# edwardyehuang/iSeg

Measured on AMD Instinct MI355X. Metric: train_images_per_sec (ConvNeXt-T+ASPP 512x512 crop, fwd+bwd+AdamW, whole job), higher is better.
Workload: dtype bf16

## Files before the change

### iseg_amd/csrc/mlp_fused.hip

```cpp
#include "common.h"
#include "iseg_hip.h"
#include "mlp_common.h"
#include <stdlib.h>

namespace {

typedef __attribute__((ext_vector_type(16))) float f32x16;
typedef __attribute__((address_space(3))) void* lds_void_ptr;
typedef const __attribute__((address_space(1))) void* glb_void_ptr;

constexpr int OUT_SLAB = 32 * 36 * 4;

template <int C, int SUB, int WAVES, int NIMG, int NSTAGES> struct MlpGeom {
    static constexpr int NS = NSTAGES;
    static constexpr int HID = 4 * C, KK = C / 16, CB = C / 32;
    static constexpr int IMG = C * 64;
    static constexpr int SLAB = NIMG * IMG;
    static constexpr int STAGE = SUB * SLAB;
    static constexpr int PIECES = STAGE / 1024;
    static constexpr int PLO = PIECES / WAVES, NHI = PIECES % WAVES, PHI = PLO + (NHI ? 1 : 0);
    static constexpr int NST = HID / (32 * SUB);
    static constexpr int RING = NS * STAGE > WAVES * OUT_SLAB ? NS * STAGE : WAVES * OUT_SLAB;
    static constexpr int LDS = RING + HID * 4;
    static_assert(C % 32 == 0 && STAGE % 1024 == 0 && HID % (32 * SUB) == 0 && PLO >= 1 && NST >= NS - 1 && NS >= 2 && LDS <= 160 * 1024, "geometry");
};

__device__ __forceinline__ bf16x8 lds_frag(const char* p) { return *reinterpret_cast<const bf16x8*>(p); }

template <class G, int WAVES> struct RingFeeder {
    const char* src;
    int wid;
    __device__ __forceinline__ RingFeeder(const void* tiled, int wid_, int lane) : src((const char*)tiled + wid_ * 1024 + lane * 16), wid(wid_) {}
    __device__ __forceinline__ void issue(char* smem, int stage) {
        char* dst = smem + stage * G::STAGE + wid * 1024;
#pragma unroll
        for (int i = 0; i < G::PLO; ++i)
            __builtin_amdgcn_global_load_lds((glb_void_ptr)(src + i * WAVES * 1024), (lds_void_ptr)(dst + i * WAVES * 1024), 16, 0, 0);
        if (G::NHI && wid < G::NHI)
            __builtin_amdgcn_global_load_lds((glb_void_ptr)(src + G::PLO * WAVES * 1024), (lds_void_ptr)(dst + G::PLO * WAVES * 1024), 16, 0, 0);
        src += G::STAGE;
    }
};


#define MLP_WAIT(N) asm volatile("s_waitcnt vmcnt(%0)" ::"n"(N) : "memory")

template <int C, int SUB, int WAVES, int NSTAGES>
__global__ __launch_bounds__(64 * WAVES) __attribute__((amdgpu_waves_per_eu(C == 96 ? 4 : (C == 192 ? 2 : 1)))) void convnext_mlp_fwd_kernel(const bf16_t* __restrict__ Y, const void* __restrict__ FW,
                                                               const float* __restrict__ b1, const float* __restrict__ b2,
                                                               const float* __restrict__ gamma, const float* __restrict__ rowscale,
                                                               int64_t rows_per_group, const bf16_t* __restrict__ R, bf16_t* __restrict__ O,
                                                               int64_t M, MlpLayerNorm ln) {
    using G = MlpGeom<C, SUB, WAVES, 2, NSTAGES>;
    constexpr int HID = G::HID, KK = G::KK, CB = G::CB, IMG = G::IMG, SLAB = G::SLAB, STAGE = G::STAGE, NST = G::NST, NS = G::NS;
    extern __shared__ __attribute__((aligned(1024))) char smem[];
    float* const b1s = reinterpret_cast<float*>(smem + G::RING);

    const int tid = threadIdx.x, lane = tid & 63, wid = tid >> 6;
    const int r = lane & 31, h = lane >> 5;
    const int64_t m0 = (int64_t)blockIdx.x * (32 * WAVES) + wid * 32;

    bf16x8 yf[KK];
    {
        int64_t row = m0 + r;
        row = row < M ? row : M - 1;
        const bf16_t* yp = Y + row * C + 8 * h;
#ifdef ISEG_ABL_MLP_NOIO
#pragma unroll
        for (int kk = 0; kk < KK; ++kk)
#pragma unroll
            for (int u = 0; u < 8; ++u) yf[kk][u] = (bf16_t)(0.01f * (float)((lane + kk + u) & 15));
        (void)yp;
#else
#pragma unroll
        for (int kk = 0; kk < KK; ++kk) yf[kk] = *reinterpret_cast<const bf16x8*>(yp + 16 * kk);
#endif
        if (ln.gamma) mlp_layernorm_rows<KK>(yf, ln, m0 + r < M ? m0 + r : -1, h, C);
    }
    for (int i = tid; i < HID; i += 64 * WAVES) b1s[i] = b1[i];
#pragma unroll
    for (int kk = 0; kk < KK; ++kk) asm volatile("" ::"v"(yf[kk]));

    RingFeeder<G, WAVES> feed(FW, wid, lane);

    f32x16 acc[CB];
#pragma unroll
    for (int cb = 0; cb < CB; ++cb)
// ... 17 lines not shown
        for (int sub = 0; sub < SUB; ++sub) {
            const int f0 = sub * (KK + 2 * CB);
            f32x16 hacc;
            {
                const float* bb = b1s + 32 * (kt * SUB + sub) + 4 * h;
#pragma unroll
                for (int i = 0; i < 4; ++i) {
                    const float4 v = __builtin_bit_cast(float4, lds_frag(reinterpret_cast<const char*>(bb + 8 * i)));
                    hacc[4 * i] = v.x;
                    hacc[4 * i + 1] = v.y;
                    hacc[4 * i + 2] = v.z;
                    hacc[4 * i + 3] = v.w;
                }
            }
#pragma unroll
            for (int kk = 0; kk < KK; ++kk) {
                hacc = __builtin_amdgcn_mfma_f32_32x32x16_bf16(take(f0 + kk), yf[kk], hacc, 0, 0, 0);
                __builtin_amdgcn_sched_barrier(0);
            }
            bf16x8 gf[2];
#pragma unroll
            for (int j = 0; j < 16; ++j) gf[j >> 3][j & 7] = (bf16_t)gelu_poly(hacc[j]);
            __builtin_amdgcn_sched_barrier(0);
#pragma unroll
            for (int cb = 0; cb < CB; ++cb)
#pragma unroll
                for (int s = 0; s < 2; ++s) {
                    acc[cb] = __builtin_amdgcn_mfma_f32_32x32x16_bf16(take(f0 + KK + 2 * cb + s), gf[s], acc[cb], 0, 0, 0);
                    __builtin_amdgcn_sched_barrier(0);
                }
        }
    };

#pragma unroll
    for (int p = 0; p < NS - 1; ++p) feed.issue(smem, p);
    int stage = 0, fill = NS - 1;
    for (int kt = 0; kt < NST; ++kt) {
        if (NST - 1 - kt >= NS - 2) {
            if (G::NHI && wid < G::NHI) MLP_WAIT((NS - 2) * G::PHI);
            else MLP_WAIT((NS - 2) * G::PLO);
        } else {
            MLP_WAIT(0);
        }
        asm volatile("s_waitcnt lgkmcnt(0)" ::: "memory");
        __builtin_amdgcn_s_barrier();
        asm volatile("" ::: "memory");
        if (kt + NS - 1 < NST) feed.issue(smem, fill);
        compute(stage, kt);
        stage = stage + 1 == NS ? 0 : stage + 1;
        fill = fill + 1 == NS ? 0 : fill + 1;
    }
    asm volatile("s_waitcnt lgkmcnt(0)" ::: "memory");
    __builtin_amdgcn_s_barrier();
    asm volatile("" ::: "memory");

    float* const slab = reinterpret_cast<float*>(smem + wid * OUT_SLAB);
    const int er = lane >> 1, eh = lane & 1;
    const int64_t m = m0 + er;
    float rs = 1.f;
    if (rowscale && m < M) rs = rowscale[m / rows_per_group];
#pragma unroll
    for (int cb = 0; cb < CB; ++cb) {
#pragma unroll
        for (int i = 0; i < 4; ++i)
            *reinterpret_cast<float4*>(slab + r * 36 + 8 * i + 4 * h) = make_float4(acc[cb][4 * i], acc[cb][4 * i + 1], acc[cb][4 * i + 2], acc[cb][4 * i + 3]);
        float v[16];
#pragma unroll
        for (int i = 0; i < 4; ++i) {
            const float4 t = *reinterpret_cast<const float4*>(slab + er * 36 + 16 * eh + 4 * i);
            v[4 * i] = t.x;
            v[4 * i + 1] = t.y;
            v[4 * i + 2] = t.z;
            v[4 * i + 3] = t.w;
        }
        if (m < M) {
            const int c0 = 32 * cb + 16 * eh;
            float res[16], bb[16], gg[16];
#ifdef ISEG_ABL_MLP_NOIO
#pragma unroll
            for (int u = 0; u < 16; ++u) res[u] = 0.f;
#else
            load8<bf16_t>(R + m * C + c0, res);
            load8<bf16_t>(R + m * C + c0 + 8, res + 8);
// ... 15 lines not shown
#endif
            {
                store8<bf16_t>(O + m * C + c0, v);
                store8<bf16_t>(O + m * C + c0 + 8, v + 8);
            }
        }
    }
}

__device__ __forceinline__ uint32_t pack_bf16x2(float lo, float hi) {
    typedef __attribute__((ext_vector_type(2))) __bf16 bf16x2;
    bf16x2 v;
    v[0] = (bf16_t)lo;
    v[1] = (bf16_t)hi;
    return __builtin_bit_cast(uint32_t, v);
}

__device__ __forceinline__ void acc_to_row_pieces(const float* v, uint4& p0, uint4& p1) {
    uint32_t d[8];
#pragma unroll
    for (int i = 0; i < 8; ++i) d[i] = pack_bf16x2(v[2 * i], v[2 * i + 1]);
#pragma unroll
    for (int pr = 0; pr < 2; ++pr)
#pragma unroll
        for (int w = 0; w < 2; ++w) {
            auto sw = __builtin_amdgcn_permlane32_swap(d[4 * pr + w], d[4 * pr + 2 + w], false, false);
            d[4 * pr + w] = sw[0];
            d[4 * pr + 2 + w] = sw[1];
        }
    p0 = make_uint4(d[0], d[1], d[2], d[3]);
    p1 = make_uint4(d[4], d[5], d[6], d[7]);
}

template <int C, int SUB, int WAVES, int NSTAGES, bool STORE, bool LNB = false>
__global__ __launch_bounds__(64 * WAVES) void convnext_mlp_bwd_kernel(const bf16_t* __restrict__ Y, const bf16_t* __restrict__ D,
                                                                      const float* __restrict__ rowscale, int64_t rows_per_group,
                                                                      const void* __restrict__ BW, const float* __restrict__ b1,
                                                                      bf16_t* __restrict__ Gout, bf16_t* __restrict__ DHout,
                                                                      bf16_t* __restrict__ DY, int64_t M, MlpLayerNorm ln,
                                                                      float* __restrict__ ln_partials) {
    using G = MlpGeom<C, SUB, WAVES, 3, NSTAGES>;
    constexpr int HID = G::HID, KK = G::KK, CB = G::CB, IMG = G::IMG, SLAB = G::SLAB, STAGE = G::STAGE, NST = G::NST, NS = G::NS;
    constexpr int STORES = STORE ? 4 * SUB : 0;
    extern __shared__ __attribute__((aligned(1024))) char smem[];
    float* const b1s = reinterpret_cast<float*>(smem + G::RING);

    const int tid = threadIdx.x, lane = tid & 63, wid = tid >> 6;
    const int r = lane & 31, h = lane >> 5;
    const int64_t m0 = (int64_t)blockIdx.x * (32 * WAVES) + wid * 32;
    const bool active = m0 < M;

    bf16x8 yf[KK], df[KK];
    {
        int64_t row = m0 + r;
        row = row < M ? row : M - 1;
        const bf16_t* yp = Y + row * C + 8 * h;
        const bf16_t* dp = D + row * C + 8 * h;
#pragma unroll
        for (int kk = 0; kk < KK; ++kk) {
            yf[kk] = *reinterpret_cast<const bf16x8*>(yp + 16 * kk);
            df[kk] = *reinterpret_cast<const bf16x8*>(dp + 16 * kk);
        }
        if (ln.gamma) mlp_layernorm_apply_rows<KK>(yf, ln, row, h);
        if (rowscale) {
            const float rs = rowscale[row / rows_per_group];
#pragma unroll
            for (int kk = 0; kk < KK; ++kk)
#pragma unroll
                for (int u = 0; u < 8; ++u) df[kk][u] = (bf16_t)((float)df[kk][u] * rs);
        }
    }
    for (int i = tid; i < HID; i += 64 * WAVES) b1s[i] = b1[i];
#pragma unroll
    for (int kk = 0; kk < KK; ++kk) asm volatile("" ::"v"(yf[kk]), "v"(df[kk]));

    RingFeeder<G, WAVES> feed(BW, wid, lane);
// ... 50 lines not shown
#pragma unroll
            for (int j = 0; j < 16; ++j) {
                float gd;
                if constexpr (STORE) gelu_sig_both(hacc[j], gv[j], gd);
                else gd = gelu_poly_grad(hacc[j]);
                dv[j] = dacc[j] * gd;
            }
            bf16x8 hf[2];
#pragma unroll
            for (int j = 0; j < 16; ++j) hf[j >> 3][j & 7] = (bf16_t)dv[j];
            __builtin_amdgcn_sched_barrier(0);
#pragma unroll
            for (int cb = 0; cb < CB; ++cb)
#pragma unroll
                for (int s = 0; s < 2; ++s) {
                    acc[cb] = __builtin_amdgcn_mfma_f32_32x32x16_bf16(take(f0 + 2 * KK + 2 * cb + s), hf[s], acc[cb], 0, 0, 0);
                    __builtin_amdgcn_sched_barrier(0);
                }
            if (STORE) {
                uint4 g0, g1, d0, d1;
                acc_to_row_pieces(gv, g0, g1);
                acc_to_row_pieces(dv, d0, d1);
                if (row_ok) {
                    const int64_t o = row_o + 32 * (kt * SUB + sub);
                    *reinterpret_cast<uint4*>(Gout + o) = g0;
                    *reinterpret_cast<uint4*>(Gout + o + 16) = g1;
                    *reinterpret_cast<uint4*>(DHout + o) = d0;
                    *reinterpret_cast<uint4*>(DHout + o + 16) = d1;
                }
            }
        }
    };

#pragma unroll
    for (int p = 0; p < NS - 1; ++p) feed.issue(smem, p);
    int stage = 0, fill = NS - 1;
    for (int kt = 0; kt < NST; ++kt) {
        {
            const bool more = NST - 1 - kt >= NS - 2;
            const bool hi = G::NHI && wid < G::NHI;
#define MLP_WAIT_BWD(S_)                                                     \
    do {                                                                     \
        if (more) {                                                          \
            if (hi) MLP_WAIT((NS - 2) * G::PHI + (S_));                      \
            else MLP_WAIT((NS - 2) * G::PLO + (S_));                         \
        } else {                                                             \
            MLP_WAIT(S_);                                                    \
        }                                                                    \
    } while (0)
            if (!active || kt == 0) MLP_WAIT_BWD(0);
            else if (kt == 1) MLP_WAIT_BWD(STORES);
            else MLP_WAIT_BWD(2 * STORES);
#undef MLP_WAIT_BWD
        }
        asm volatile("s_waitcnt lgkmcnt(0)" ::: "memory");
        __builtin_amdgcn_s_barrier();
        asm volatile("" ::: "memory");
        if (kt + NS - 1 < NST) feed.issue(smem, fill);
        if (active) compute(stage, kt);
        stage = stage + 1 == NS ? 0 : stage + 1;
        fill = fill + 1 == NS ? 0 : fill + 1;
    }
    asm volatile("s_waitcnt lgkmcnt(0)" ::: "memory");
    __builtin_amdgcn_s_barrier();
    asm volatile("" ::: "memory");

    float* const slab = reinterpret_cast<float*>(smem + wid * OUT_SLAB);
    const int er = lane >> 1, eh = lane & 1;
    const int64_t m = m0 + er;
    auto exchange = [&](int cb, float* v) {
#pragma unroll
        for (int i = 0; i < 4; ++i)
            *reinterpret_cast<float4*>(slab + r * 36 + 8 * i + 4 * h) = make_float4(acc[cb][4 * i], acc[cb][4 * i + 1], acc[cb][4 * i + 2], acc[cb][4 * i + 3]);
#pragma unroll
        for (int i = 0; i < 4; ++i) {
            const float4 t = *reinterpret_cast<const float4*>(slab + er * 36 + 16 * eh + 4 * i);
            v[4 * i] = t.x;
            v[4 * i + 1] = t.y;
            v[4 * i + 2] = t.z;
            v[4 * i + 3] = t.w;
        }
    };
    if constexpr (!LNB) {
#pragma unroll
        for (int cb = 0; cb < CB; ++cb) {
            float v[16];
            exchange(cb, v);
            if (m < M) {
                const int c0 = 32 * cb + 16 * eh;
                store8<bf16_t>(DY + m * C + c0, v);
                store8<bf16_t>(DY + m * C + c0 + 8, v + 8);
            }
        }
    } else {
// ... 122 lines not shown
__global__ void convnext_weight_prep_batched_kernel(const int64_t* __restrict__ table) {
    const int64_t* e = table + 8 * blockIdx.y;
    const int first = blockIdx.x * blockDim.x + threadIdx.x, stride = gridDim.x * blockDim.x;
    if (e[0] == 1) {
        mlp_prep_elements(reinterpret_cast<const float*>(e[1]), reinterpret_cast<const float*>(e[2]), reinterpret_cast<const float*>(e[3]),
                          reinterpret_cast<bf16_t*>(e[4]), reinterpret_cast<bf16_t*>(e[5]), (int)e[6], first, stride);
    } else if (e[0] == 2) {
        const float* wa = reinterpret_cast<const float*>(e[1]);
        const float* wb = reinterpret_cast<const float*>(e[2]);
        const float* ba = reinterpret_cast<const float*>(e[3]);
        const float* bb = reinterpret_cast<const float*>(e[5]);
        const int Cc = (int)e[6], na = (int)(e[7] & 0xFFFFF), nb = (int)((e[7] >> 20) & 0xFFFFF), ld = (int)(e[7] >> 40);
        bf16_t* rowcat = reinterpret_cast<bf16_t*>(e[4]);
        bf16_t* tr = rowcat + (int64_t)Cc * ld;
        float* bias = reinterpret_cast<float*>(tr + (int64_t)Cc * ld);
        const int64_t total = (int64_t)Cc * ld;
        for (int64_t i = first; i < total; i += stride) {
            const int c = (int)(i / ld), j = (int)(i % ld);
            const float v = j < na ? wa[(int64_t)c * na + j] : (j < na + nb ? wb[(int64_t)c * nb + (j - na)] : 0.f);
            rowcat[i] = (bf16_t)v;
            tr[(int64_t)j * Cc + c] = (bf16_t)v;
        }
        for (int j = first; j < ld; j += stride) bias[j] = j < na ? (ba ? ba[j] : 0.f) : (j < na + nb ? (bb ? bb[j - na] : 0.f) : 0.f);
    } else {
        const float* src = reinterpret_cast<const float*>(e[1]);
        const float* g = reinterpret_cast<const float*>(e[3]);
        bf16_t* dst = reinterpret_cast<bf16_t*>(e[4]);
        const int cols = (int)e[6];
        const int64_t total = e[7] * cols;
        for (int64_t i = first; i < total; i += stride) dst[i] = (bf16_t)(src[i] * g[i % cols]);
    }
}

template <int C, int SUB, int WAVES, int NSTAGES>
int launch_mlp_fwd(const void* y2, const void* FW, const float* b1, const float* b2, const float* gamma, const float* rowscale,
                   int64_t rows_per_group, const void* residual, void* out, int64_t M, const MlpLayerNorm& ln, hipStream_t s) {
    using G = MlpGeom<C, SUB, WAVES, 2, NSTAGES>;
    static const bool raised = [] {
        return hipFuncSetAttribute(reinterpret_cast<const void*>(&convnext_mlp_fwd_kernel<C, SUB, WAVES, NSTAGES>),
                                   hipFuncAttributeMaxDynamicSharedMemorySize, G::LDS) == hipSuccess;
    }();
    (void)raised;
    const int grid = (int)ceil_div64(M, 32 * WAVES);
    hipLaunchKernelGGL((convnext_mlp_fwd_kernel<C, SUB, WAVES, NSTAGES>), dim3(grid), dim3(64 * WAVES), G::LDS, s, (const bf16_t*)y2, FW, b1, b2, gamma, rowscale,
                       rows_per_group, (const bf16_t*)residual, (bf16_t*)out, M, ln);
    return iseg_check_launch("iseg_convnext_mlp_fwd");
}

template <int C, int SUB, int WAVES, int NSTAGES, bool STORE, bool LNB = false>
int launch_mlp_bwd(const void* y2, const void* dbr, const float* rowscale, int64_t rows_per_group, const void* BW, const float* b1, void* g,
                   void* dh, void* dy2, int64_t M, const MlpLayerNorm& ln, hipStream_t s, float* ln_partials = nullptr) {
    using G = MlpGeom<C, SUB, WAVES, 3, NSTAGES>;
    static_assert(!LNB || G::RING >= WAVES * OUT_SLAB + (WAVES * 2 + 1) * C * 4, "the column sums and gamma sit behind the epilogue slabs inside the ring");
    static const bool raised = [] {
        return hipFuncSetAttribute(reinterpret_cast<const void*>(&convnext_mlp_bwd_kernel<C, SUB, WAVES, NSTAGES, STORE, LNB>),
                                   hipFuncAttributeMaxDynamicSharedMemorySize, G::LDS) == hipSuccess;
    }();
    (void)raised;
    const int grid = (int)ceil_div64(M, 32 * WAVES);
    hipLaunchKernelGGL((convnext_mlp_bwd_kernel<C, SUB, WAVES, NSTAGES, STORE, LNB>), dim3(grid), dim3(64 * WAVES), G::LDS, s, (const bf16_t*)y2,
                       (const bf16_t*)dbr, rowscale, rows_per_group, BW, b1, (bf16_t*)g, (bf16_t*)dh, (bf16_t*)dy2, M, ln, ln_partials);
    return iseg_check_launch("iseg_convnext_mlp_bwd");
}

}

extern "C" int iseg_convnext_mlp_supported(int C, int dtype) {
    static const bool wide = [] { const char* e = getenv("ISEG_MLP_FUSED_384"); return e && atoi(e) != 0; }();
    return dtype == ISEG_BF16 && (C == 96 || C == 192 || (C == 384 && wide)) ? 1 : 0;
}

extern "C" size_t iseg_convnext_mlp_tiled_bytes(int C, int backward) { return (size_t)(backward ? 3 : 2) * 4 * C * C * 2; }

extern "C" int iseg_convnext_mlp_prep(const float* W1, const float* W2, const float* gamma, void* fw_tiled, void* bw_tiled, int C,
                                      hipStream_t stream) {
    ISEG_REQUIRE(W1 && W2 && fw_tiled && C > 0 && C % 32 == 0, "iseg_convnext_mlp_prep: bad arguments");
    const int total = (bw_tiled ? 5 : 2) * 4 * C * C;
    hipLaunchKernelGGL(convnext_mlp_prep_kernel, dim3((total + 255) / 256), dim3(256), 0, stream, W1, W2, gamma, (bf16_t*)fw_tiled,
                       (bf16_t*)bw_tiled, C);
    return iseg_check_launch("iseg_convnext_mlp_prep");
}

extern "C" int iseg_convnext_weight_prep_batched(const int64_t* table, int entries, int64_t max_elements, hipStream_t stream) {
    ISEG_REQUIRE(table && entries > 0 && max_elements > 0, "iseg_convnext_weight_prep_batched: bad arguments");
    int64_t bx = (max_elements + 255) / 256;
    if (bx > 256) bx = 256;
    hipLaunchKernelGGL(convnext_weight_prep_batched_kernel, dim3((unsigned)bx, (unsigned)entries), dim3(256), 0, stream, table);
    return iseg_check_launch("iseg_convnext_weight_prep_batched");
}

extern "C" int iseg_convnext_mlp_fwd(const void* y2, const void* fw_tiled, const float* b1, const float* b2, const float* gamma,
                                     const float* rowscale, int64_t rows_per_group, const void* residual, void* out, int64_t M, int C, int dtype,
                                     hipStream_t stream) {
    ISEG_REQUIRE(iseg_convnext_mlp_supported(C, dtype), "iseg_convnext_mlp_fwd: bf16 storage with C = 96, 192 or 384 only (C = %d, dtype = %d)", C, dtype);
    ISEG_REQUIRE(y2 && fw_tiled && b1 && b2 && residual && out && M > 0, "iseg_convnext_mlp_fwd: null operand or empty problem");
    ISEG_REQUIRE(!rowscale || rows_per_group > 0, "iseg_convnext_mlp_fwd: rowscale needs rows_per_group > 0");
    ISEG_REQUIRE((((uintptr_t)y2 | (uintptr_t)fw_tiled | (uintptr_t)residual | (uintptr_t)out | (uintptr_t)b1 | (uintptr_t)b2 | (uintptr_t)gamma) & 15) == 0,
                 "iseg_convnext_mlp_fwd: operands must be 16-byte aligned");
    const MlpLayerNorm none{};
    if (C == 96) return launch_mlp_fwd<96, 2, 8, 3>(y2, fw_tiled, b1, b2, gamma, rowscale, rows_per_group, residual, out, M, none, stream);
    if (C == 192) return launch_mlp_fwd<192, 1, 8, 3>(y2, fw_tiled, b1, b2, gamma, rowscale, rows_per_group, residual, out, M, none, stream);
    return launch_mlp_fwd<384, 1, 4, 3>(y2, fw_tiled, b1, b2, gamma, rowscale, rows_per_group, residual, out, M, none, stream);
}

extern "C" int iseg_convnext_mlp_fwd_ln(const void* y1, const float* ln_gamma, const float* ln_beta, float eps, float* mean, float* rstd,
                                        const void* fw_tiled, const float* b1, const float* b2, const float* gamma, const float* rowscale,
                                        int64_t rows_per_group, const void* residual, void* out, int64_t M, int C, int dtype, hipStream_t stream) {
    ISEG_REQUIRE(dtype == ISEG_BF16 && (C == 96 || C == 192), "iseg_convnext_mlp_fwd_ln: bf16 storage with C = 96 or 192 only (C = %d, dtype = %d)", C, dtype);
    ISEG_REQUIRE(y1 && ln_gamma && ln_beta && mean && rstd && fw_tiled && b1 && b2 && residual && out && M > 0,
                 "iseg_convnext_mlp_fwd_ln: null operand or empty problem");
    ISEG_REQUIRE(!rowscale || rows_per_group > 0, "iseg_convnext_mlp_fwd_ln: rowscale needs rows_per_group > 0");
    ISEG_REQUIRE((((uintptr_t)y1 | (uintptr_t)fw_tiled | (uintptr_t)residual | (uintptr_t)out | (uintptr_t)b1 | (uintptr_t)b2 | (uintptr_t)gamma |
                   (uintptr_t)ln_gamma | (uintptr_t)ln_beta) & 15) == 0, "iseg_convnext_mlp_fwd_ln: operands must be 16-byte aligned");
    const MlpLayerNorm ln{ln_gamma, ln_beta, mean, rstd, eps};
    if (C == 96) return launch_mlp_fwd<96, 2, 8, 3>(y1, fw_tiled, b1, b2, gamma, rowscale, rows_per_group, residual, out, M, ln, stream);
    return launch_mlp_fwd<192, 1, 8, 3>(y1, fw_tiled, b1, b2, gamma, rowscale, rows_per_group, residual, out, M, ln, stream);
}

extern "C" int iseg_convnext_mlp_bwd(const void* y2, const void* dbr, const void* bw_tiled, const float* b1, void* g, void* dh, void* dy2,
                                     int64_t M, int C, int dtype, hipStream_t stream) {
    ISEG_REQUIRE(iseg_convnext_mlp_supported(C, dtype), "iseg_convnext_mlp_bwd: bf16 storage with C = 96, 192 or 384 only (C = %d, dtype = %d)", C, dtype);
    ISEG_REQUIRE(y2 && dbr && bw_tiled && b1 && g && dh && dy2 && M > 0, "iseg_convnext_mlp_bwd: null operand or empty problem");
    ISEG_REQUIRE((((uintptr_t)y2 | (uintptr_t)dbr | (uintptr_t)bw_tiled | (uintptr_t)b1 | (uintptr_t)g | (uintptr_t)dh | (uintptr_t)dy2) & 15) == 0,
                 "iseg_convnext_mlp_bwd: operands must be 16-byte aligned");
    const MlpLayerNorm none{};
    if (C == 96) return launch_mlp_bwd<96, 2, 8, 3, true>(y2, dbr, nullptr, 0, bw_tiled, b1, g, dh, dy2, M, none, stream);
    if (C == 192) return launch_mlp_bwd<192, 1, 4, 3, true>(y2, dbr, nullptr, 0, bw_tiled, b1, g, dh, dy2, M, none, stream);
    return launch_mlp_bwd<384, 1, 4, 2, true>(y2, dbr, nullptr, 0, bw_tiled, b1, g, dh, dy2, M, none, stream);
}

extern "C" int iseg_convnext_mlp_bwd_data(const void* y2, const float* mean, const float* rstd, const float* ln_gamma, const float* ln_beta,
                                          const void* dout, const float* rowscale, int64_t rows_per_group, const void* bw_tiled,
                                          const float* b1, void* dy2, int64_t M, int C, int dtype, hipStream_t stream) {
    ISEG_REQUIRE(dtype == ISEG_BF16 && (C == 96 || C == 192), "iseg_convnext_mlp_bwd_data: bf16 storage with C = 96 or 192 only (C = %d, dtype = %d)", C, dtype);
    ISEG_REQUIRE(y2 && dout && bw_tiled && b1 && dy2 && M > 0, "iseg_convnext_mlp_bwd_data: null operand or empty problem");
    ISEG_REQUIRE(!rowscale || rows_per_group > 0, "iseg_convnext_mlp_bwd_data: rowscale needs rows_per_group > 0");
    ISEG_REQUIRE((((uintptr_t)y2 | (uintptr_t)dout | (uintptr_t)bw_tiled | (uintptr_t)b1 | (uintptr_t)dy2) & 15) == 0,
                 "iseg_convnext_mlp_bwd_data: operands must be 16-byte aligned");
    ISEG_REQUIRE(!mean || (rstd && ln_gamma && ln_beta && (((uintptr_t)ln_gamma | (uintptr_t)ln_beta) & 15) == 0),
                 "iseg_convnext_mlp_bwd_data: mean needs rstd and 16-byte aligned ln_gamma / ln_beta");
    const MlpLayerNorm ln{mean ? ln_gamma : nullptr, ln_beta, const_cast<float*>(mean), const_cast<float*>(rstd), 0.f};
    if (C == 96) return launch_mlp_bwd<96, 2, 8, 3, false>(y2, dout, rowscale, rows_per_group, bw_tiled, b1, nullptr, nullptr, dy2, M, ln, stream);
    return launch_mlp_bwd<192, 1, 4, 3, false>(y2, dout, rowscale, rows_per_group, bw_tiled, b1, nullptr, nullptr, dy2, M, ln, stream);
}

static int64_t mlp_bwd_blocks(int64_t M, int C) { return ceil_div64(M, 32 * (C == 96 ? 8 : 4)); }

extern "C" size_t iseg_convnext_mlp_bwd_data_ln_workspace_bytes(int64_t M, int C) {
    return (C == 96 || C == 192) && M > 0 ? (size_t)mlp_bwd_blocks(M, C) * 2 * C * sizeof(float) : 0;
}

extern "C" int iseg_convnext_mlp_bwd_data_ln(const void* y1, const float* mean, const float* rstd, const float* ln_gamma, const float* ln_beta,
                                             const void* dout, const float* rowscale, int64_t rows_per_group, const void* bw_tiled,
                                             const float* b1, void* dy1, float* dln_gamma, float* dln_beta, int64_t M, int C, int dtype,
                                             void* ws, size_t ws_bytes, hipStream_t stream) {
    ISEG_REQUIRE(dtype == ISEG_BF16 && (C == 96 || C == 192), "iseg_convnext_mlp_bwd_data_ln: bf16 storage with C = 96 or 192 only (C = %d, dtype = %d)", C, dtype);
    ISEG_REQUIRE(y1 && mean && rstd && ln_gamma && ln_beta && dout && bw_tiled && b1 && dy1 && dln_gamma && dln_beta && M > 0,
                 "iseg_convnext_mlp_bwd_data_ln: null operand or empty problem");
    ISEG_REQUIRE(!rowscale || rows_per_group > 0, "iseg_convnext_mlp_bwd_data_ln: rowscale needs rows_per_group > 0");
    ISEG_REQUIRE((((uintptr_t)y1 | (uintptr_t)dout | (uintptr_t)bw_tiled | (uintptr_t)b1 | (uintptr_t)dy1 | (uintptr_t)ln_gamma | (uintptr_t)ln_beta) & 15) == 0,
                 "iseg_convnext_mlp_bwd_data_ln: operands must be 16-byte aligned");
    const size_t need = iseg_convnext_mlp_bwd_data_ln_workspace_bytes(M, C);
    if (!ws || ws_bytes < need) {
        iseg_set_error("iseg_convnext_mlp_bwd_data_ln: needs %zu workspace bytes, got %zu", need, ws_bytes);
        return ISEG_ERR_WORKSPACE;
    }
    const MlpLayerNorm ln{ln_gamma, ln_beta, const_cast<float*>(mean), const_cast<float*>(rstd), 0.f};
    float* partials = (float*)ws;
    float* const arena = iseg_deferred_partials(need, dln_gamma, dln_beta, 1, stream);
    if (arena) partials = arena;
    const int rc = C == 96 ? launch_mlp_bwd<96, 2, 8, 3, false, true>(y1, dout, rowscale, rows_per_group, bw_tiled, b1, nullptr, nullptr, dy1, M, ln,
                                                                       stream, partials)
                           : launch_mlp_bwd<192, 1, 4, 3, false, true>(y1, dout, rowscale, rows_per_group, bw_tiled, b1, nullptr, nullptr, dy1, M, ln,
                                                                        stream, partials);
    if (rc != ISEG_OK) return rc;
    const int blocks = (int)mlp_bwd_blocks(M, C);
    if (arena) iseg_deferred_push(partials, blocks, 2 * C, 2 * C, dln_gamma, dln_beta, C, 1.f, stream);
    else launch_reduce_rows(partials, blocks, 2 * C, 0, 1, 2 * C, dln_gamma, dln_beta, C, 0, 1.f, 1, stream);
    return iseg_check_launch("iseg_convnext_mlp_bwd_data_ln");
}
```

Measured before the change: 1938.

## Skew fused ConvNeXt MLP pipeline to overlap GELU with next slab's MFMAs

Adds a software-pipelined (skewed) schedule to the fused ConvNeXt MLP forward and backward-data kernels. The first-layer product for the next hidden slab is issued while the GELU (or GELU-gradient) of the current slab runs, interleaved with sched_group_barrier hints, so VALU work hides behind MFMA latency. The ring-wait logic is generalized into a helper to cover reading two ring stages per iteration. The new path is on by default for C=192 forward and for backward-data, and is gated by an environment variable. The forward C=96 variant needs level 2 and also lowers the waves-per-EU hint when enabled. The cost is extra registers for the second accumulator, which may lower occupancy.

```diff
diff --git a/iseg_amd/csrc/mlp_fused.hip b/iseg_amd/csrc/mlp_fused.hip
--- a/iseg_amd/csrc/mlp_fused.hip
+++ b/iseg_amd/csrc/mlp_fused.hip
@@ -45,14 +45,65 @@
 
 #define MLP_WAIT(N) asm volatile("s_waitcnt vmcnt(%0)" ::"n"(N) : "memory")
 
-template <int C, int SUB, int WAVES, int NSTAGES>
-__global__ __launch_bounds__(64 * WAVES) __attribute__((amdgpu_waves_per_eu(C == 96 ? 4 : (C == 192 ? 2 : 1)))) void convnext_mlp_fwd_kernel(const bf16_t* __restrict__ Y, const void* __restrict__ FW,
+template <class G, int STORES, int MAXP> __device__ __forceinline__ void mlp_ring_wait(int stages, int store_iters, bool hi) {
+#define MLP_WAIT_PK(P_, K_)                                                          \
+    do {                                                                             \
+        if (hi) MLP_WAIT((P_ * G::PHI + K_ * STORES) < 63 ? P_ * G::PHI + K_ * STORES : 63); \
+        else MLP_WAIT((P_ * G::PLO + K_ * STORES) < 63 ? P_ * G::PLO + K_ * STORES : 63);    \
+    } while (0)
+#define MLP_WAIT_P(P_)                                  \
+    do {                                                \
+        if (STORES == 0 || store_iters == 0) MLP_WAIT_PK(P_, 0); \
+        else if (store_iters == 1) MLP_WAIT_PK(P_, 1);  \
+        else MLP_WAIT_PK(P_, 2);                        \
+    } while (0)
+    if (MAXP == 0 || stages == 0) MLP_WAIT_P(0);
+    else if (MAXP == 1 || stages == 1) MLP_WAIT_P(1);
+    else MLP_WAIT_P(2);
+#undef MLP_WAIT_P
+#undef MLP_WAIT_PK
+}
+
+template <class G, int STORES, bool SKEW> __device__ __forceinline__ void mlp_ring_sync(int kt, bool stores_issued) {
+    constexpr int NS = G::NS, NST = G::NST;
+    const int need = SKEW && kt + 1 < NST ? kt + 1 : kt;
+    const int issued = kt + NS - 2 < NST - 1 ? kt + NS - 2 : NST - 1;
+    const int first_store = need - (NS - 1) > 0 ? need - (NS - 1) : 0;
+    int k = stores_issued && STORES ? kt - first_store : 0;
+    k = k < 2 ? k : 2;
+    constexpr int MAXP = (SKEW ? NS - 3 : NS - 2) < 2 ? (SKEW ? NS - 3 : NS - 2) : 2;
+    static_assert(NS <= 4 || !SKEW, "mlp_ring_wait counts at most two pending stages");
+    mlp_ring_wait<G, STORES, MAXP>(issued - need, k, G::NHI && threadIdx.x / 64 < G::NHI);
+    asm volatile("s_waitcnt lgkmcnt(0)" ::: "memory");
+    __builtin_amdgcn_s_barrier();
+    asm volatile("" ::: "memory");
+}
+
+template <bool B> struct MlpFlag { static constexpr bool value = B; };
+
+#ifndef ISEG_MLP_SKEW_NS
+#define ISEG_MLP_SKEW_NS 3
+#endif
+#ifndef ISEG_MLP_SKEW_ALT
+#define ISEG_MLP_SKEW_ALT 0
+#endif
+
+constexpr int SG_VALU = 0x2, SG_MFMA = 0x8, SG_DS_READ = 0x100;
+#ifdef ISEG_MLP_NOSGB
+#define MLP_SGB(M_, N_) ((void)0)
+#else
+#define MLP_SGB(M_, N_) __builtin_amdgcn_sched_group_barrier(M_, N_, 0)
+#endif
+
+template <int C, int SUB, int WAVES, int NSTAGES, bool SKEW>
+__global__ __launch_bounds__(64 * WAVES) __attribute__((amdgpu_waves_per_eu(C == 96 ? (SKEW ? 2 : 4) : (C == 192 ? 2 : 1)))) void convnext_mlp_fwd_kernel(const bf16_t* __restrict__ Y, const void* __restrict__ FW,
                                                                const float* __restrict__ b1, const float* __restrict__ b2,
                                                                const float* __restrict__ gamma, const float* __restrict__ rowscale,
                                                                int64_t rows_per_group, const bf16_t* __restrict__ R, bf16_t* __restrict__ O,
                                                                int64_t M, MlpLayerNorm ln) {
     using G = MlpGeom<C, SUB, WAVES, 2, NSTAGES>;
     constexpr int HID = G::HID, KK = G::KK, CB = G::CB, IMG = G::IMG, SLAB = G::SLAB, STAGE = G::STAGE, NST = G::NST, NS = G::NS;
+    static_assert(!SKEW || (NS >= 3 && NST >= 2), "the skewed schedule reads two ring stages per iteration and refills a third");
     extern __shared__ __attribute__((aligned(1024))) char smem[];
     float* const b1s = reinterpret_cast<float*>(smem + G::RING);
 
@@ -136,23 +187,123 @@
         }
     };
 
+    constexpr int PER = KK + 2 * CB;
+#ifndef ISEG_MLP_SKEW_FD
+#define ISEG_MLP_SKEW_FD FD
+#endif
+    constexpr int FDS = ISEG_MLP_SKEW_FD;
+    constexpr int VALU_A = 16 * 11 + 8;
+    constexpr int VPER = (VALU_A + KK) / (KK + 1) + 11;
+    f32x16 hc;
+    auto bias = [&](int slab) {
+        f32x16 a;
+        const float* bb = b1s + 32 * slab + 4 * h;
+#pragma unroll
+        for (int i = 0; i < 4; ++i) {
+            const float4 v = __builtin_bit_cast(float4, lds_frag(reinterpret_cast<const char*>(bb + 8 * i)));
+            a[4 * i] = v.x;
+            a[4 * i + 1] = v.y;
+            a[4 * i + 2] = v.z;
+            a[4 * i + 3] = v.w;
+        }
+        return a;
+    };
+    auto first_product = [&](int stage) {
+        const char* fb = smem + stage * STAGE + fo;
+        bf16x8 win[FDS];
+#pragma unroll
+        for (int d = 0; d < FDS; ++d) win[d] = lds_frag(fb + d * 1024);
+        hc = bias(0);
+#pragma unroll
+        for (int kk = 0; kk < KK; ++kk) {
+            const bf16x8 a = win[kk % FDS];
+            if (kk + FDS < KK) win[kk % FDS] = lds_frag(fb + (kk + FDS) * 1024);
+            hc = __builtin_amdgcn_mfma_f32_32x32x16_bf16(a, yf[kk], hc, 0, 0, 0);
+            __builtin_amdgcn_sched_barrier(0);
+        }
+    };
+    auto compute_skew = [&](int stage, int kt, auto last_c) {
+        constexpr bool LAST = decltype(last_c)::value;
+        constexpr int NFS = SUB * PER - (LAST ? KK : 0);
+        const char* cur = smem + stage * STAGE + fo;
+        const char* nxt = smem + (stage + 1 == NS ? 0 : stage + 1) * STAGE + fo;
+        auto frag_at = [&](int f) {
+            const int sub = f / PER, q = f % PER;
+            const bool succ = !(LAST && sub == SUB - 1);
+            if (succ && q < KK) return lds_frag((sub + 1 < SUB ? cur + (sub + 1) * SLAB : nxt) + q * 1024);
+            return lds_frag(cur + sub * SLAB + (succ ? q : KK + q) * 1024);
+        };
+        bf16x8 win[FDS];
+#pragma unroll
+        for (int d = 0; d < FDS; ++d) win[d] = frag_at(d);
+        auto take = [&](int f) {
+            const bf16x8 a = win[f % FDS];
+            if (f + FDS < NFS) win[f % FDS] = frag_at(f + FDS);
+            return a;
+        };
+#pragma unroll
+        for (int sub = 0; sub < SUB; ++sub) {
+            const int f0 = sub * PER;
+            const bool succ = !(LAST && sub == SUB - 1);
+            bf16x8 gf[2];
+            if (succ) {
+                f32x16 hn = bias(kt * SUB + sub + 1);
+                __builtin_amdgcn_sched_barrier(0);
+#pragma unroll
+                for (int c = 0; c <= KK; ++c) {
+                    if (c > 0) hn = __builtin_amdgcn_mfma_f32_32x32x16_bf16(take(f0 + c - 1), yf[c - 1], hn, 0, 0, 0);
+#pragma unroll
+                    for (int j = 16 * c / (KK + 1); j < 16 * (c + 1) / (KK + 1); ++j) gf[j >> 3][j & 7] = (bf16_t)gelu_poly(hc[j]);
+                    if (c > 0) {
+                        MLP_SGB(SG_MFMA, 1);
+                        MLP_SGB(SG_DS_READ, 1);
+                        MLP_SGB(SG_VALU, VPER);
+                    }
+                    __builtin_amdgcn_sched_barrier(0);
+                }
+                hc = hn;
+            } else {
+#pragma unroll
+                for (int j = 0; j < 16; ++j) gf[j >> 3][j & 7] = (bf16_t)gelu_poly(hc[j]);
+                __builtin_amdgcn_sched_barrier(0);
+            }
+            const int f2 = f0 + (succ ? KK : 0);
+#pragma unroll
+            for (int cb = 0; cb < CB; ++cb)
+#pragma unroll
+                for (int s = 0; s < 2; ++s) {
+                    acc[cb] = __builtin_amdgcn_mfma_f32_32x32x16_bf16(take(f2 + 2 * cb + s), gf[s], acc[cb], 0, 0, 0);
+                    __builtin_amdgcn_sched_barrier(0);
+                }
+        }
+    };
+
 #pragma unroll
     for (int p = 0; p < NS - 1; ++p) feed.issue(smem, p);
     int stage = 0, fill = NS - 1;
-    for (int kt = 0; kt < NST; ++kt) {
-        if (NST - 1 - kt >= NS - 2) {
-            if (G::NHI && wid < G::NHI) MLP_WAIT((NS - 2) * G::PHI);
-            else MLP_WAIT((NS - 2) * G::PLO);
-        } else {
-            MLP_WAIT(0);
-        }
-        asm volatile("s_waitcnt lgkmcnt(0)" ::: "memory");
-        __builtin_amdgcn_s_barrier();
-        asm volatile("" ::: "memory");
-        if (kt + NS - 1 < NST) feed.issue(smem, fill);
-        compute(stage, kt);
-        stage = stage + 1 == NS ? 0 : stage + 1;
-        fill = fill + 1 == NS ? 0 : fill + 1;
+    if constexpr (SKEW) {
+        mlp_ring_sync<G, 0, true>(0, false);
+        if (NS - 1 < NST) feed.issue(smem, fill);
+        first_product(stage);
+        compute_skew(stage, 0, MlpFlag<false>{});
+        stage = 1, fill = 0;
+        for (int kt = 1; kt < NST - 1; ++kt) {
+            mlp_ring_sync<G, 0, true>(kt, false);
+            if (kt + NS - 1 < NST) feed.issue(smem, fill);
+            compute_skew(stage, kt, MlpFlag<false>{});
+            stage = stage + 1 == NS ? 0 : stage + 1;
+            fill = fill + 1 == NS ? 0 : fill + 1;
+        }
+        mlp_ring_sync<G, 0, true>(NST - 1, false);
+        compute_skew(stage, NST - 1, MlpFlag<true>{});
+    } else {
+        for (int kt = 0; kt < NST; ++kt) {
+            mlp_ring_sync<G, 0, false>(kt, false);
+            if (kt + NS - 1 < NST) feed.issue(smem, fill);
+            compute(stage, kt);
+            stage = stage + 1 == NS ? 0 : stage + 1;
+            fill = fill + 1 == NS ? 0 : fill + 1;
+        }
     }
     asm volatile("s_waitcnt lgkmcnt(0)" ::: "memory");
     __builtin_amdgcn_s_barrier();
@@ -234,7 +385,7 @@
     p1 = make_uint4(d[4], d[5], d[6], d[7]);
 }
 
-template <int C, int SUB, int WAVES, int NSTAGES, bool STORE, bool LNB = false>
+template <int C, int SUB, int WAVES, int NSTAGES, bool STORE, bool LNB, bool SKEW>
 __global__ __launch_bounds__(64 * WAVES) void convnext_mlp_bwd_kernel(const bf16_t* __restrict__ Y, const bf16_t* __restrict__ D,
                                                                       const float* __restrict__ rowscale, int64_t rows_per_group,
                                                                       const void* __restrict__ BW, const float* __restrict__ b1,
@@ -244,6 +395,7 @@
     using G = MlpGeom<C, SUB, WAVES, 3, NSTAGES>;
     constexpr int HID = G::HID, KK = G::KK, CB = G::CB, IMG = G::IMG, SLAB = G::SLAB, STAGE = G::STAGE, NST = G::NST, NS = G::NS;
     constexpr int STORES = STORE ? 4 * SUB : 0;
+    static_assert(!SKEW || (NS >= 3 && NST >= 2), "the skewed schedule reads two ring stages per iteration and refills a third");
     extern __shared__ __attribute__((aligned(1024))) char smem[];
     float* const b1s = reinterpret_cast<float*>(smem + G::RING);
 
@@ -360,34 +512,148 @@
         }
     };
 
+    constexpr int NP1 = 2 * KK, PER = NP1 + 2 * CB;
+    constexpr bool ALT = ISEG_MLP_SKEW_ALT;
+    constexpr int VALU_A = STORE ? 16 * 24 + 8 : 16 * 13 + 8;
+    constexpr int VPER = (VALU_A + NP1) / (NP1 + 1) + 24;
+    f32x16 hc, dc;
+    auto bias = [&](int slab) {
+        f32x16 a;
+        const float* bb = b1s + 32 * slab + 4 * h;
+#pragma unroll
+        for (int i = 0; i < 4; ++i) {
+            const float4 v = __builtin_bit_cast(float4, lds_frag(reinterpret_cast<const char*>(bb + 8 * i)));
+            a[4 * i] = v.x;
+            a[4 * i + 1] = v.y;
+            a[4 * i + 2] = v.z;
+            a[4 * i + 3] = v.w;
+        }
+        return a;
+    };
+    auto first_product = [&](int stage) {
+        const char* fb = smem + stage * STAGE + fo;
+        bf16x8 win[FD];
+#pragma unroll
+        for (int d = 0; d < FD; ++d) win[d] = lds_frag(fb + d * 1024);
+        hc = bias(0);
+#pragma unroll
+        for (int j = 0; j < 16; ++j) dc[j] = 0.f;
+#pragma unroll
+        for (int f = 0; f < NP1; ++f) {
+            const bf16x8 a = win[f % FD];
+            if (f + FD < NP1) win[f % FD] = lds_frag(fb + (f + FD) * 1024);
+            if (f < KK) hc = __builtin_amdgcn_mfma_f32_32x32x16_bf16(a, yf[f], hc, 0, 0, 0);
+            else dc = __builtin_amdgcn_mfma_f32_32x32x16_bf16(a, df[f - KK], dc, 0, 0, 0);
+            __builtin_amdgcn_sched_barrier(0);
+        }
+    };
+    auto compute_skew = [&](int stage, int kt, auto last_c) {
+        constexpr bool LAST = decltype(last_c)::value;
+        constexpr int NFS = SUB * PER - (LAST ? NP1 : 0);
+        const char* cur = smem + stage * STAGE + fo;
+        const char* nxt = smem + (stage + 1 == NS ? 0 : stage + 1) * STAGE + fo;
+        auto frag_at = [&](int f) {
+            const int sub = f / PER, q = f % PER;
+            const bool succ = !(LAST && sub == SUB - 1);
+            if (succ && q < NP1) return lds_frag((sub + 1 < SUB ? cur + (sub + 1) * SLAB : nxt) + (ALT ? (q & 1 ? KK : 0) + q / 2 : q) * 1024);
+            return lds_frag(cur + sub * SLAB + (succ ? q : NP1 + q) * 1024);
+        };
+        bf16x8 win[FD];
+#pragma unroll
+        for (int d = 0; d < FD; ++d) win[d] = frag_at(d);
+        auto take = [&](int f) {
+            const bf16x8 a = win[f % FD];
+            if (f + FD < NFS) win[f % FD] = frag_at(f + FD);
+            return a;
+        };
+#pragma unroll
+        for (int sub = 0; sub < SUB; ++sub) {
+            const int f0 = sub * PER;
+            const bool succ = !(LAST && sub == SUB - 1);
+            float gv[16], dv[16];
+            bf16x8 hf[2];
+            auto chain = [&](int j0, int j1) {
+#pragma unroll
+                for (int j = j0; j < j1; ++j) {
+                    float gd;
+                    if constexpr (STORE) gelu_sig_both(hc[j], gv[j], gd);
+                    else gd = gelu_poly_grad(hc[j]);
+                    dv[j] = dc[j] * gd;
+                    hf[j >> 3][j & 7] = (bf16_t)dv[j];
+                }
+            };
+            if (succ) {
+                f32x16 hn = bias(kt * SUB + sub + 1), dn;
+#pragma unroll
+                for (int j = 0; j < 16; ++j) dn[j] = 0.f;
+                __builtin_amdgcn_sched_barrier(0);
+#pragma unroll
+                for (int c = 0; c <= NP1; ++c) {
+                    const int f = c - 1, kh = ALT ? f / 2 : f;
+                    if (c > 0 && (ALT ? (f & 1) == 0 : f < KK)) hn = __builtin_amdgcn_mfma_f32_32x32x16_bf16(take(f0 + f), yf[kh], hn, 0, 0, 0);
+                    if (c > 0 && (ALT ? (f & 1) == 1 : f >= KK)) dn = __builtin_amdgcn_mfma_f32_32x32x16_bf16(take(f0 + f), df[ALT ? kh : f - KK], dn, 0, 0, 0);
+                    chain(16 * c / (NP1 + 1), 16 * (c + 1) / (NP1 + 1));
+                    if (c > 0) {
+                        MLP_SGB(SG_MFMA, 1);
+                        MLP_SGB(SG_DS_READ, 1);
+                        MLP_SGB(SG_VALU, VPER);
+                    }
+                    __builtin_amdgcn_sched_barrier(0);
+                }
+                hc = hn;
+                dc = dn;
+            } else {
+                chain(0, 16);
+                __builtin_amdgcn_sched_barrier(0);
+            }
+            const int f2 = f0 + (succ ? NP1 : 0);
+#pragma unroll
+            for (int cb = 0; cb < CB; ++cb)
+#pragma unroll
+                for (int s = 0; s < 2; ++s) {
+                    acc[cb] = __builtin_amdgcn_mfma_f32_32x32x16_bf16(take(f2 + 2 * cb + s), hf[s], acc[cb], 0, 0, 0);
+                    __builtin_amdgcn_sched_barrier(0);
+                }
+            if (STORE) {
+                uint4 g0, g1, d0, d1;
+                acc_to_row_pieces(gv, g0, g1);
+                acc_to_row_pieces(dv, d0, d1);
+                if (row_ok) {
+                    const int64_t o = row_o + 32 * (kt * SUB + sub);
+                    *reinterpret_cast<uint4*>(Gout + o) = g0;
+                    *reinterpret_cast<uint4*>(Gout + o + 16) = g1;
+                    *reinterpret_cast<uint4*>(DHout + o) = d0;
+                    *reinterpret_cast<uint4*>(DHout + o + 16) = d1;
+                }
+            }
+        }
+    };
+
 #pragma unroll
     for (int p = 0; p < NS - 1; ++p) feed.issue(smem, p);
     int stage = 0, fill = NS - 1;
-    for (int kt = 0; kt < NST; ++kt) {
-        {
-            const bool more = NST - 1 - kt >= NS - 2;
-            const bool hi = G::NHI && wid < G::NHI;
-#define MLP_WAIT_BWD(S_)                                                     \
-    do {                                                                     \
-        if (more) {                                                          \
-            if (hi) MLP_WAIT((NS - 2) * G::PHI + (S_));                      \
-            else MLP_WAIT((NS - 2) * G::PLO + (S_));                         \
-        } else {                                                             \
-            MLP_WAIT(S_);                                                    \
-        }                                                                    \
-    } while (0)
-            if (!active || kt == 0) MLP_WAIT_BWD(0);
-            else if (kt == 1) MLP_WAIT_BWD(STORES);
-            else MLP_WAIT_BWD(2 * STORES);
-#undef MLP_WAIT_BWD
-        }
-        asm volatile("s_waitcnt lgkmcnt(0)" ::: "memory");
-        __builtin_amdgcn_s_barrier();
-        asm volatile("" ::: "memory");
+    if constexpr (SKEW) {
+        mlp_ring_sync<G, STORES, true>(0, active);
+        if (NS - 1 < NST) feed.issue(smem, fill);
+        if (active) {
+            first_product(stage);
+            compute_skew(stage, 0, MlpFlag<false>{});
+        }
+        stage = 1, fill = 0;
+    }
+    for (int kt = SKEW ? 1 : 0; kt < (SKEW ? NST - 1 : NST); ++kt) {
+        mlp_ring_sync<G, STORES, SKEW>(kt, active);
         if (kt + NS - 1 < NST) feed.issue(smem, fill);
-        if (active) compute(stage, kt);
+        if (active) {
+            if constexpr (SKEW) compute_skew(stage, kt, MlpFlag<false>{});
+            else compute(stage, kt);
+        }
         stage = stage + 1 == NS ? 0 : stage + 1;
         fill = fill + 1 == NS ? 0 : fill + 1;
+    }
+    if constexpr (SKEW) {
+        mlp_ring_sync<G, STORES, true>(NST - 1, active);
+        if (active) compute_skew(stage, NST - 1, MlpFlag<true>{});
     }
     asm volatile("s_waitcnt lgkmcnt(0)" ::: "memory");
     __builtin_amdgcn_s_barrier();
@@ -576,36 +842,43 @@
     }
 }
 
-template <int C, int SUB, int WAVES, int NSTAGES>
+template <int C, int SUB, int WAVES, int NSTAGES, bool SKEW>
 int launch_mlp_fwd(const void* y2, const void* FW, const float* b1, const float* b2, const float* gamma, const float* rowscale,
                    int64_t rows_per_group, const void* residual, void* out, int64_t M, const MlpLayerNorm& ln, hipStream_t s) {
     using G = MlpGeom<C, SUB, WAVES, 2, NSTAGES>;
     static const bool raised = [] {
-        return hipFuncSetAttribute(reinterpret_cast<const void*>(&convnext_mlp_fwd_kernel<C, SUB, WAVES, NSTAGES>),
+        return hipFuncSetAttribute(reinterpret_cast<const void*>(&convnext_mlp_fwd_kernel<C, SUB, WAVES, NSTAGES, SKEW>),
                                    hipFuncAttributeMaxDynamicSharedMemorySize, G::LDS) == hipSuccess;
     }();
     (void)raised;
     const int grid = (int)ceil_div64(M, 32 * WAVES);
-    hipLaunchKernelGGL((convnext_mlp_fwd_kernel<C, SUB, WAVES, NSTAGES>), dim3(grid), dim3(64 * WAVES), G::LDS, s, (const bf16_t*)y2, FW, b1, b2, gamma, rowscale,
+    hipLaunchKernelGGL((convnext_mlp_fwd_kernel<C, SUB, WAVES, NSTAGES, SKEW>), dim3(grid), dim3(64 * WAVES), G::LDS, s, (const bf16_t*)y2, FW, b1, b2, gamma, rowscale,
                        rows_per_group, (const bf16_t*)residual, (bf16_t*)out, M, ln);
     return iseg_check_launch("iseg_convnext_mlp_fwd");
 }
 
-template <int C, int SUB, int WAVES, int NSTAGES, bool STORE, bool LNB = false>
+template <int C, int SUB, int WAVES, int NSTAGES, bool STORE, bool LNB, bool SKEW>
 int launch_mlp_bwd(const void* y2, const void* dbr, const float* rowscale, int64_t rows_per_group, const void* BW, const float* b1, void* g,
                    void* dh, void* dy2, int64_t M, const MlpLayerNorm& ln, hipStream_t s, float* ln_partials = nullptr) {
     using G = MlpGeom<C, SUB, WAVES, 3, NSTAGES>;
     static_assert(!LNB || G::RING >= WAVES * OUT_SLAB + (WAVES * 2 + 1) * C * 4, "the column sums and gamma sit behind the epilogue slabs inside the ring");
     static const bool raised = [] {
-        return hipFuncSetAttribute(reinterpret_cast<const void*>(&convnext_mlp_bwd_kernel<C, SUB, WAVES, NSTAGES, STORE, LNB>),
+        return hipFuncSetAttribute(reinterpret_cast<const void*>(&convnext_mlp_bwd_kernel<C, SUB, WAVES, NSTAGES, STORE, LNB, SKEW>),
                                    hipFuncAttributeMaxDynamicSharedMemorySize, G::LDS) == hipSuccess;
     }();
     (void)raised;
     const int grid = (int)ceil_div64(M, 32 * WAVES);
-    hipLaunchKernelGGL((convnext_mlp_bwd_kernel<C, SUB, WAVES, NSTAGES, STORE, LNB>), dim3(grid), dim3(64 * WAVES), G::LDS, s, (const bf16_t*)y2,
+    hipLaunchKernelGGL((convnext_mlp_bwd_kernel<C, SUB, WAVES, NSTAGES, STORE, LNB, SKEW>), dim3(grid), dim3(64 * WAVES), G::LDS, s, (const bf16_t*)y2,
                        (const bf16_t*)dbr, rowscale, rows_per_group, BW, b1, (bf16_t*)g, (bf16_t*)dh, (bf16_t*)dy2, M, ln, ln_partials);
     return iseg_check_launch("iseg_convnext_mlp_bwd");
 }
+
+int mlp_skew_level() {
+    static const int lvl = [] { const char* e = getenv("ISEG_MLP_SKEW"); return e ? atoi(e) : 1; }();
+    return lvl;
+}
+bool mlp_skew() { return mlp_skew_level() != 0; }
+bool mlp_skew_fwd96() { return mlp_skew_level() >= 2; }
 
 }
 
@@ -642,9 +915,14 @@
     ISEG_REQUIRE((((uintptr_t)y2 | (uintptr_t)fw_tiled | (uintptr_t)residual | (uintptr_t)out | (uintptr_t)b1 | (uintptr_t)b2 | (uintptr_t)gamma) & 15) == 0,
                  "iseg_convnext_mlp_fwd: operands must be 16-byte aligned");
     const MlpLayerNorm none{};
-    if (C == 96) return launch_mlp_fwd<96, 2, 8, 3>(y2, fw_tiled, b1, b2, gamma, rowscale, rows_per_group, residual, out, M, none, stream);
-    if (C == 192) return launch_mlp_fwd<192, 1, 8, 3>(y2, fw_tiled, b1, b2, gamma, rowscale, rows_per_group, residual, out, M, none, stream);
-    return launch_mlp_fwd<384, 1, 4, 3>(y2, fw_tiled, b1, b2, gamma, rowscale, rows_per_group, residual, out, M, none, stream);
+    const bool skew = mlp_skew();
+    if (C == 96)
+        return mlp_skew_fwd96() ? launch_mlp_fwd<96, 2, 8, ISEG_MLP_SKEW_NS, true>(y2, fw_tiled, b1, b2, gamma, rowscale, rows_per_group, residual, out, M, none, stream)
+                    : launch_mlp_fwd<96, 2, 8, 3, false>(y2, fw_tiled, b1, b2, gamma, rowscale, rows_per_group, residual, out, M, none, stream);
+    if (C == 192)
+        return skew ? launch_mlp_fwd<192, 1, 8, ISEG_MLP_SKEW_NS, true>(y2, fw_tiled, b1, b2, gamma, rowscale, rows_per_group, residual, out, M, none, stream)
+                    : launch_mlp_fwd<192, 1, 8, 3, false>(y2, fw_tiled, b1, b2, gamma, rowscale, rows_per_group, residual, out, M, none, stream);
+    return launch_mlp_fwd<384, 1, 4, 3, false>(y2, fw_tiled, b1, b2, gamma, rowscale, rows_per_group, residual, out, M, none, stream);
 }
 
 extern "C" int iseg_convnext_mlp_fwd_ln(const void* y1, const float* ln_gamma, const float* ln_beta, float eps, float* mean, float* rstd,
@@ -657,8 +935,12 @@
     ISEG_REQUIRE((((uintptr_t)y1 | (uintptr_t)fw_tiled | (uintptr_t)residual | (uintptr_t)out | (uintptr_t)b1 | (uintptr_t)b2 | (uintptr_t)gamma |
                    (uintptr_t)ln_gamma | (uintptr_t)ln_beta) & 15) == 0, "iseg_convnext_mlp_fwd_ln: operands must be 16-byte aligned");
     const MlpLayerNorm ln{ln_gamma, ln_beta, mean, rstd, eps};
-    if (C == 96) return launch_mlp_fwd<96, 2, 8, 3>(y1, fw_tiled, b1, b2, gamma, rowscale, rows_per_group, residual, out, M, ln, stream);
-    return launch_mlp_fwd<192, 1, 8, 3>(y1, fw_tiled, b1, b2, gamma, rowscale, rows_per_group, residual, out, M, ln, stream);
+    const bool skew = mlp_skew();
+    if (C == 96)
+        return mlp_skew_fwd96() ? launch_mlp_fwd<96, 2, 8, ISEG_MLP_SKEW_NS, true>(y1, fw_tiled, b1, b2, gamma, rowscale, rows_per_group, residual, out, M, ln, stream)
+                    : launch_mlp_fwd<96, 2, 8, 3, false>(y1, fw_tiled, b1, b2, gamma, rowscale, rows_per_group, residual, out, M, ln, stream);
+    return skew ? launch_mlp_fwd<192, 1, 8, ISEG_MLP_SKEW_NS, true>(y1, fw_tiled, b1, b2, gamma, rowscale, rows_per_group, residual, out, M, ln, stream)
+                : launch_mlp_fwd<192, 1, 8, 3, false>(y1, fw_tiled, b1, b2, gamma, rowscale, rows_per_group, residual, out, M, ln, stream);
 }
 
 extern "C" int iseg_convnext_mlp_bwd(const void* y2, const void* dbr, const void* bw_tiled, const float* b1, void* g, void* dh, void* dy2,
@@ -668,9 +950,9 @@
     ISEG_REQUIRE((((uintptr_t)y2 | (uintptr_t)dbr | (uintptr_t)bw_tiled | (uintptr_t)b1 | (uintptr_t)g | (uintptr_t)dh | (uintptr_t)dy2) & 15) == 0,
                  "iseg_convnext_mlp_bwd: operands must be 16-byte aligned");
     const MlpLayerNorm none{};
-    if (C == 96) return launch_mlp_bwd<96, 2, 8, 3, true>(y2, dbr, nullptr, 0, bw_tiled, b1, g, dh, dy2, M, none, stream);
-    if (C == 192) return launch_mlp_bwd<192, 1, 4, 3, true>(y2, dbr, nullptr, 0, bw_tiled, b1, g, dh, dy2, M, none, stream);
-    return launch_mlp_bwd<384, 1, 4, 2, true>(y2, dbr, nullptr, 0, bw_tiled, b1, g, dh, dy2, M, none, stream);
+    if (C == 96) return launch_mlp_bwd<96, 2, 8, 3, true, false, false>(y2, dbr, nullptr, 0, bw_tiled, b1, g, dh, dy2, M, none, stream);
+    if (C == 192) return launch_mlp_bwd<192, 1, 4, 3, true, false, false>(y2, dbr, nullptr, 0, bw_tiled, b1, g, dh, dy2, M, none, stream);
+    return launch_mlp_bwd<384, 1, 4, 2, true, false, false>(y2, dbr, nullptr, 0, bw_tiled, b1, g, dh, dy2, M, none, stream);
 }
 
 extern "C" int iseg_convnext_mlp_bwd_data(const void* y2, const float* mean, const float* rstd, const float* ln_gamma, const float* ln_beta,
@@ -684,8 +966,12 @@
     ISEG_REQUIRE(!mean || (rstd && ln_gamma && ln_beta && (((uintptr_t)ln_gamma | (uintptr_t)ln_beta) & 15) == 0),
                  "iseg_convnext_mlp_bwd_data: mean needs rstd and 16-byte aligned ln_gamma / ln_beta");
     const MlpLayerNorm ln{mean ? ln_gamma : nullptr, ln_beta, const_cast<float*>(mean), const_cast<float*>(rstd), 0.f};
-    if (C == 96) return launch_mlp_bwd<96, 2, 8, 3, false>(y2, dout, rowscale, rows_per_group, bw_tiled, b1, nullptr, nullptr, dy2, M, ln, stream);
-    return launch_mlp_bwd<192, 1, 4, 3, false>(y2, dout, rowscale, rows_per_group, bw_tiled, b1, nullptr, nullptr, dy2, M, ln, stream);
+    const bool skew = mlp_skew();
+    if (C == 96)
+        return skew ? launch_mlp_bwd<96, 2, 8, ISEG_MLP_SKEW_NS, false, false, true>(y2, dout, rowscale, rows_per_group, bw_tiled, b1, nullptr, nullptr, dy2, M, ln, stream)
+                    : launch_mlp_bwd<96, 2, 8, 3, false, false, false>(y2, dout, rowscale, rows_per_group, bw_tiled, b1, nullptr, nullptr, dy2, M, ln, stream);
+    return skew ? launch_mlp_bwd<192, 1, 4, ISEG_MLP_SKEW_NS, false, false, true>(y2, dout, rowscale, rows_per_group, bw_tiled, b1, nullptr, nullptr, dy2, M, ln, stream)
+                : launch_mlp_bwd<192, 1, 4, 3, false, false, false>(y2, dout, rowscale, rows_per_group, bw_tiled, b1, nullptr, nullptr, dy2, M, ln, stream);
 }
 
 static int64_t mlp_bwd_blocks(int64_t M, int C) { return ceil_div64(M, 32 * (C == 96 ? 8 : 4)); }
@@ -713,10 +999,14 @@
     float* partials = (float*)ws;
     float* const arena = iseg_deferred_partials(need, dln_gamma, dln_beta, 1, stream);
     if (arena) partials = arena;
-    const int rc = C == 96 ? launch_mlp_bwd<96, 2, 8, 3, false, true>(y1, dout, rowscale, rows_per_group, bw_tiled, b1, nullptr, nullptr, dy1, M, ln,
-                                                                       stream, partials)
-                           : launch_mlp_bwd<192, 1, 4, 3, false, true>(y1, dout, rowscale, rows_per_group, bw_tiled, b1, nullptr, nullptr, dy1, M, ln,
-                                                                        stream, partials);
+    const bool skew = mlp_skew();
+    int rc;
+    if (C == 96)
+        rc = skew ? launch_mlp_bwd<96, 2, 8, ISEG_MLP_SKEW_NS, false, true, true>(y1, dout, rowscale, rows_per_group, bw_tiled, b1, nullptr, nullptr, dy1, M, ln, stream, partials)
+                  : launch_mlp_bwd<96, 2, 8, 3, false, true, false>(y1, dout, rowscale, rows_per_group, bw_tiled, b1, nullptr, nullptr, dy1, M, ln, stream, partials);
+    else
+        rc = skew ? launch_mlp_bwd<192, 1, 4, ISEG_MLP_SKEW_NS, false, true, true>(y1, dout, rowscale, rows_per_group, bw_tiled, b1, nullptr, nullptr, dy1, M, ln, stream, partials)
+                  : launch_mlp_bwd<192, 1, 4, 3, false, true, false>(y1, dout, rowscale, rows_per_group, bw_tiled, b1, nullptr, nullptr, dy1, M, ln, stream, partials);
     if (rc != ISEG_OK) return rc;
     const int blocks = (int)mlp_bwd_blocks(M, C);
     if (arena) iseg_deferred_push(partials, blocks, 2 * C, 2 * C, dln_gamma, dln_beta, C, 1.f, stream);
```

Result: no change. 1941 (median of 6 runs) (+0.2%).
